# megvii-research/basedet

Hardware: AMD Instinct MI355X
Metric: images/sec training RetinaNet-R50-FPN 1333x800 (higher is better)
Workload: dtype bf16; 1 GPU; retinanet_r50_800x1344 train step (fwd+bwd+allreduce+SGD), DummyLoader boxes, random-init weights, inputs resident in HBM; per_gpu_batch=16, global_batch=16, parallelism=dp1

## Files before the change

### basedet_amd/_lib.py

```python
import ctypes as C
import os

import torch

_HERE = os.path.dirname(os.path.abspath(__file__))
LIB_PATH = os.environ.get("BASEDET_HIP_LIB") or os.path.join(_HERE, "lib", "libbasedet_hip.so")

BD_MAX_SEGS = 8
ABI_VERSION = 118
EPI_RELU, EPI_ADD_BEFORE, EPI_ADD_AFTER, EPI_MASK, EPI_SPARSE = 1, 2, 4, 8, 16


class BasedetHipError(RuntimeError):
    pass


class ConvDesc(C.Structure):
    _fields_ = [
        ("N", C.c_int32), ("Cin", C.c_int32), ("Cout", C.c_int32), ("R", C.c_int32), ("S", C.c_int32),
        ("stride", C.c_int32), ("pad", C.c_int32), ("nseg", C.c_int32),
        ("Hi", C.c_int32 * BD_MAX_SEGS), ("Wi", C.c_int32 * BD_MAX_SEGS),
        ("Ho", C.c_int32 * BD_MAX_SEGS), ("Wo", C.c_int32 * BD_MAX_SEGS),
        ("in_off", C.c_int32 * BD_MAX_SEGS), ("out_off", C.c_int32 * BD_MAX_SEGS),
        ("in_pix_per_img", C.c_int32), ("out_pix_per_img", C.c_int32),
# ... 98 lines not shown
    "bd_box_encode": (_I, [_P, _P, _L, _P, _P, _P, _P]),
    "bd_box_decode": (_I, [_P, _P, _L, _P, _P, _P, _P]),
    "bd_retina_assign_encode": (_I, [_P, _I, _P, _P, _I, _I, _F, _F, _I, _P, _P, _P, _P, _P, _P, _P, _Z, _P]),
    "bd_fcos_assign": (_I, [_P, _I, _P, _P, _P, _I, _F, _P, _P, _I, _I, _P, _P, _P, _P, _P]),
    "bd_ota_assign_workspace_bytes": (_Z, [_I, _I]),
    "bd_ota_assign": (_I, [_P, _I, _P, _P, _I, _P, _I, _I, _P, _P, _P, _I, _I, _F, _F, _F, _F, _I, _P, _P, _P, _P, _P, _Z, _P]),
    "bd_ota_sinkhorn_workspace_bytes": (_Z, [_I, _I, _I]),
    "bd_ota_assign_sinkhorn": (_I, [_P, _I, _P, _P, _I, _P, _I, _I, _P, _P, _P, _I, _I, _F, _F, _F, _F, _I, _F, _I, _P, _P, _P, _P, _P, _Z, _P]),
    "bd_freeanchor_workspace_bytes": (_Z, [_I, _I, _I, _I]),
    "bd_freeanchor_loss_fwd_bwd": (_I, [_P, _I, _P, _I, _I, _P, _I, _I, _P, _P, _I, _I, _P, _P, _F, _I, _F, _F, _F, _F, _P, _P, _P, _P, _Z, _P]),
    "bd_atss_assign_workspace_bytes": (_Z, [_I, _I]),
    "bd_atss_assign": (_I, [_P, _I, _P, _P, _I, _I, _F, _P, _P, _I, _I, _P, _P, _P, _P, _P, _Z, _P]),
    "bd_nms_workspace_bytes": (_Z, [_I]),
    "bd_batched_nms": (_I, [_P, _P, _P, _I, _F, _I, _P, _P, _P, _Z, _P]),
    "bd_focal_loss_fwd_bwd": (_I, [_P, _P, _L, _I, _I, _F, _F, _P, _I, _F, _P, _P, _I, _P]),
    "bd_smooth_l1_fwd_bwd": (_I, [_P, _P, _P, _L, _I, _I, _F, _P, _I, _F, _P, _P, _P]),
    "bd_loss_grid_cap": (_I, []),
    "bd_iou_ltrb_fwd_bwd": (_I, [_P, _P, _P, _P, _L, _I, _P, _F, _P, _P, _P]),
    "bd_bce_logits_fwd_bwd": (_I, [_P, _I, _I, _P, _P, _L, _P, _P, _P, _P]),
    "bd_groupnorm_workspace_bytes": (_Z, [_I, _I, _I, _L]),
    "bd_groupnorm_fwd": (_I, [_P, _P, _P, _I, _I, _P, _P, _L, _I, _F, _I, _P, _P, _P, _Z, _P]),
    "bd_conv2d_fwd_gnstats_bytes": (_Z, [_D]),
    "bd_conv2d_fwd_gnstats": (_I, [_D, _P, _P, _P, _P, _P, _Z, _P]),
    "bd_groupnorm_fwd_parts": (_I, [_D, _P, _P, _P, _P, _F, _I, _P, _P, _P]),
    "bd_groupnorm_bwd": (_I, [_P, _P, _P, _P, _P, _I, _I, _P, _P, _L, _I, _I, _P, _P, _P, _I, _P, _Z, _P]),
    "bd_bn_workspace_bytes": (_Z, [_L, _I]),
    "bd_bn_stats_fwd": (_I, [_P, _I, _L, _L, _L, _I, _F, _F, _P, _P, _P, _P, _P, _P, _Z, _P]),
    "bd_bn_apply_act_fwd": (_I, [_P, _L, _L, _P, _P, _P, _P, _P, _L, _L, _P, _L, _L, _I, _L, _I, _I, _P]),
    "bd_bn_bwd_reduce": (_I, [_P, _L, _L, _P, _L, _L, _P, _P, _I, _L, _I, _P, _P, _P, _Z, _P]),
    "bd_bn_bwd_apply": (_I, [_P, _L, _L, _P, _L, _L, _P, _P, _P, _P, _P, _P, _P, _L, _L, _I, _L, _I, _P]),
    "bd_bn_silu_fwd": (_I, [_P, _L, _L, _P, _P, _P, _P, _P, _L, _L, _I, _L, _I, _P]),
# ... 151 lines not shown
```

### basedet_amd/csrc/conv3x3_pp.hip

```cpp
#include "conv3x3_pp128_body.h"

namespace {

constexpr int PH = 4, PW = 16, IH = PH + 2, IW = PW + 2;
constexpr int NPATCH = 4;
constexpr int XROWS = NPATCH * IH * IW;
constexpr int X_PITCH = 144;
constexpr int X_BYTES = XROWS * X_PITCH;
constexpr int XPASSES = 7;
constexpr int TILE_CO = 256;
constexpr int W_SLOT = TILE_CO * 128;
constexpr int NSLOT = 3;
constexpr int W_BYTES = NSLOT * W_SLOT;
constexpr int GTAB_TILES = 16;
constexpr int GTAB_BYTES = GTAB_TILES * NPATCH * 32;
constexpr int LDS_BYTES = W_BYTES + X_BYTES + TILE_CO * 4 + GTAB_BYTES;
constexpr int MAX_SEG = BD_MAX_SEGS;
constexpr int TAIL_CO = 64;

struct PSeg { int patch_start, H, W, pw, src_off, dst_off; float inv_pw; };

struct PParams {
    const bf16_raw* src;
    const bf16_raw* w;
// ... 607 lines not shown
    }
    if (!SPARSE && blockIdx.x == 0 && threadIdx.x == 0) bd_clk_mark(g_pp_clk, true);
#ifdef BD_PP_STAMP
    if (st_on) { g_pp_stamp[63] = __builtin_amdgcn_s_memrealtime(); g_pp_stamp[61] = __builtin_amdgcn_s_memtime(); }
    if (threadIdx.x == 0 && blockIdx.x < 1024) { asm volatile("s_waitcnt vmcnt(0)" ::: "memory"); g_pp_span[2 * blockIdx.x + 1] = __builtin_amdgcn_s_memrealtime(); }
#endif
}

}

BD_KNOB int g_pp_tail_split = 1;
BD_KNOB int g_pp_persistent = 1;
extern BD_KNOB int g_patch_pp;
int bd_gskip_patches(const bd_conv_desc* d, int ph, int pw);
void bd_gskip_fill(const bd_conv_desc* d, int side, const void* t, const int* live_in, int* map, hipStream_t stream);
void bd_gskip_scan(const bd_conv_desc* d, const void* g, int ph, int pw, int* mask, hipStream_t stream);
void bd_gskip_compact(const bd_conv_desc* d, int ph, int pw, const int* mask, int* live, int* list, int* count, hipStream_t stream);

extern "C" size_t bd_conv2d_dgrad_gskip_bytes(const bd_conv_desc* d) {
    if (!d || d->nseg < 1 || d->nseg > BD_MAX_SEGS || !(d->R == 3 && d->S == 3 && d->stride == 1 && d->pad == 1)) return 0;
    return ((size_t)3 * bd_gskip_patches(d, PH, PW) + 4) * sizeof(int);
}

static bool pp_sparse_epilogue(int flags, const void* add, const void* dst) {
    const bool in_place = (flags & BD_EPI_ADD_BEFORE) && add && add == dst;
    return !(flags & BD_EPI_ADD_AFTER) && (!((flags & BD_EPI_ADD_BEFORE) && add) || (in_place && !(flags & BD_EPI_MASK)));
}

bool bd_conv3x3_pp_maps_ok(const bd_conv_desc* d, int flags, const void* add, const void* dst) {
    if (g_patch_pp < 2 || !(d->R == 3 && d->S == 3 && d->stride == 1 && d->pad == 1)) return false;
    if (d->Cout % 8 != 0 || d->Cin <= 128 || d->Cin % 8 != 0) return false;
    if ((long long)d->N * d->out_pix_per_img * d->Cout * 2 >= 0x7fffffffll || (long long)d->N * d->in_pix_per_img >= 0x7fffffffll ||
// ... 80 lines not shown
        (void)hipFuncSetAttribute(reinterpret_cast<const void*>(&conv3x3_pp_kernel<0, false, true>), hipFuncAttributeMaxDynamicSharedMemorySize,
                                  LDS_BYTES));
    bd_note_kernel("conv3x3_pp_kernel");
    if (sparse) {
        const int tot = p.total_patches;
        p.sp_keep_dead = in_place ? 1 : 0;
        p.sp_stride = tot;
        if (d->gskip_gmap) {
            BdGskipMap gm;
            bd_gskip_map_layout(d, 0, &gm);
            const int* m = (const int*)d->gskip_gmap;
            p.sp_hdr = m; p.sp_live = m + gm.live; p.sp_list = m + gm.list;
        } else {
            int* mk = (int*)d->gskip_ws;
            p.sp_live = mk + tot; p.sp_list = mk + 2 * tot; p.sp_count = mk + 3 * tot;
            bd_gskip_scan(d, src, PH, PW, mk, stream);
            bd_gskip_compact(d, PH, PW, mk, mk + tot, mk + 2 * tot, mk + 3 * tot, stream);
        }
        if (d->gskip_dxmap) {
            BdGskipMap xm;
            bd_gskip_map_layout(d, 1, &xm);
            p.sp_ohdr = (int*)d->gskip_dxmap; p.sp_olist = p.sp_ohdr + xm.list;
            p.sp_clean = d->gskip_dx_clean ? 1 : 0;
        }
        hipLaunchKernelGGL((conv3x3_pp_kernel<1, false, true>), dim3(p.main_grid), dim3(512), LDS_BYTES, stream, p);
        if (d->gskip_dxmap) bd_gskip_fill(d, 1, dst, p.sp_live, (int*)d->gskip_dxmap, stream);
    } else if (fsparse) {
        const int tot = p.total_patches;
        BdFwdMap fm;
        bd_fwd_map_layout(d, &fm);
        int* m = (int*)d->fwd_map;
        p.sp_hdr = m; p.sp_live = m + fm.live; p.sp_list = m + fm.list; p.sp_stride = tot;
// ... 63 lines not shown
```

### basedet_amd/csrc/gskip.hip

```cpp
#include "common.h"

namespace {

enum { GS_ANY = 1, GS_TOP = 2, GS_BOT = 4, GS_LEFT = 8, GS_RIGHT = 16, GS_TL = 32, GS_TR = 64, GS_BL = 128, GS_BR = 256 };

struct GsSeg { int patch_start, H, W, pw, off; };

struct GsParams {
    const bf16_raw* g;
    int* mask;
    int C, ppi, ph, pw_px, nseg, patches_per_img, total;
    GsSeg seg[BD_MAX_SEGS];
};

__device__ __forceinline__ int gs_level(const GsParams& p, int rem) {
    int s = 0;
#pragma unroll
    for (int k = 1; k < BD_MAX_SEGS; ++k)
        if (k < p.nseg && rem >= p.seg[k].patch_start) s = k;
    return s;
}

__global__ __launch_bounds__(256) void gskip_scan_kernel(const GsParams p) {
    __shared__ int sbits;
    const int tid = threadIdx.x;
    const int pid = blockIdx.x;
    const int n = pid / p.patches_per_img, rem = pid - n * p.patches_per_img;
    const int s = gs_level(p, rem);
    const int H = p.seg[s].H, W = p.seg[s].W, pwn = p.seg[s].pw;
    const int local = rem - p.seg[s].patch_start, by = local / pwn, bx = local - by * pwn;
    const int y0 = by * p.ph, x0 = bx * p.pw_px;
    const int cpp = p.C >> 3;
    const int items = p.ph * p.pw_px * cpp;
    const long long img = (long long)n * p.ppi + p.seg[s].off;
    if (tid == 0) sbits = 0;
    __syncthreads();
    int bits = 0;
    constexpr int U = 8;
    for (int b = 0; b < items; b += 256 * U) {
// ... 16 lines not shown
        }
#pragma unroll
        for (int k = 0; k < U; ++k) {
            if (pix[k] >= 0 && (v[k][0] | v[k][1] | v[k][2] | v[k][3])) {
                const int py = pix[k] / p.pw_px, pxx = pix[k] - py * p.pw_px;
                const bool t = py == 0, bo = py == p.ph - 1, l = pxx == 0, r = pxx == p.pw_px - 1;
                bits |= GS_ANY | (t ? GS_TOP : 0) | (bo ? GS_BOT : 0) | (l ? GS_LEFT : 0) | (r ? GS_RIGHT : 0) | (t && l ? GS_TL : 0) |
                        (t && r ? GS_TR : 0) | (bo && l ? GS_BL : 0) | (bo && r ? GS_BR : 0);
            }
        }
    }
#pragma unroll
    for (int m = 32; m >= 1; m >>= 1) bits |= __shfl_xor(bits, m, 64);
    if ((tid & 63) == 0 && bits) atomicOr(&sbits, bits);
    __syncthreads();
    if (tid == 0) p.mask[pid] = sbits;
}

template <bool FRESH>
__device__ __forceinline__ int gs_mask(const int* m, int i) {
    if (FRESH) return __hip_atomic_load(m + i, __ATOMIC_RELAXED, __HIP_MEMORY_SCOPE_AGENT);
    return m[i];
}

template <bool FRESH>
__device__ __forceinline__ void gs_compact_body(const GsParams& p, int* live, int* list, int* count, int* wsum) {
    constexpr int KP = 8;
    const int tid = threadIdx.x, wv = tid >> 6, ln = tid & 63;
    int base = 0;
    for (int c0 = 0; c0 < p.total; c0 += 1024 * KP) {
        int lv[KP];
#pragma unroll
        for (int j = 0; j < KP; ++j) {
            const int q = c0 + tid * KP + j;
            lv[j] = 0;
            if (q < p.total) {
                const int n = q / p.patches_per_img, rem = q - n * p.patches_per_img;
                const int s = gs_level(p, rem);
                const int pwn = p.seg[s].pw, rows = (p.seg[s].H + p.ph - 1) / p.ph;
                const int local = rem - p.seg[s].patch_start, by = local / pwn, bx = local - by * pwn;
                const int* m = p.mask + (long long)n * p.patches_per_img + p.seg[s].patch_start;
                const bool up = by > 0, dn = by + 1 < rows, lf = bx > 0, rt = bx + 1 < pwn;
                int v = gs_mask<FRESH>(m, by * pwn + bx) & GS_ANY;
                if (up) v |= gs_mask<FRESH>(m, (by - 1) * pwn + bx) & GS_BOT;
                if (dn) v |= gs_mask<FRESH>(m, (by + 1) * pwn + bx) & GS_TOP;
// ... 7 lines not shown
            }
        }
        int cnt = 0;
#pragma unroll
        for (int j = 0; j < KP; ++j) cnt += lv[j];
        int inc = cnt;
#pragma unroll
        for (int o = 1; o < 64; o <<= 1) {
            const int y = __shfl_up(inc, o, 64);
            if (ln >= o) inc += y;
        }
        if (ln == 63) wsum[wv] = inc;
        __syncthreads();
        int off = base + inc - cnt, tot = 0;
#pragma unroll
        for (int w = 0; w < 16; ++w) {
            off += w < wv ? wsum[w] : 0;
            tot += wsum[w];
        }
#pragma unroll
        for (int j = 0; j < KP; ++j) {
            const int q = c0 + tid * KP + j;
            if (q < p.total) live[q] = lv[j];
            if (lv[j]) list[off++] = q;
        }
        base += tot;
        __syncthreads();
    }
    if (tid == 0) *count = base;
}

__global__ __launch_bounds__(1024) void gskip_compact_kernel(const GsParams p, int* live, int* list, int* count) {
    __shared__ int wsum[16];
    gs_compact_body<false>(p, live, list, count, wsum);
}

enum { GM_HDR = 8 };

struct GmSeg { int H, W, off, s4, s8, ss; };

struct GmParams {
    const bf16_raw* t;
    const int* live_in;
    int* map;
    int C, ppi, nseg, pi4, pi8, pis, tot4, tot8;
    GmSeg seg[BD_MAX_SEGS];
};

__global__ __launch_bounds__(1024) void gskip_fill_kernel(const GmParams p, const GsParams cp, int total) {
// ... 190 lines not shown

int bd_gskip_patches(const bd_conv_desc* d, int ph, int pw) {
    return gs_params(d, ph, pw).total;
}

void bd_gskip_scan(const bd_conv_desc* d, const void* g, int ph, int pw, int* mask, hipStream_t stream) {
    GsParams p = gs_params(d, ph, pw);
    p.g = (const bf16_raw*)g; p.mask = mask;
    if (p.total > 0) hipLaunchKernelGGL(gskip_scan_kernel, dim3(p.total), dim3(256), 0, stream, p);
}

void bd_gskip_compact(const bd_conv_desc* d, int ph, int pw, const int* mask, int* live, int* list, int* count, hipStream_t stream) {
    GsParams p = gs_params(d, ph, pw);
    p.mask = const_cast<int*>(mask);
    hipLaunchKernelGGL(gskip_compact_kernel, dim3(1), dim3(1024), 0, stream, p, live, list, count);
}

void bd_gskip_map_layout(const bd_conv_desc* d, int side, BdGskipMap* out) {
    const int p4 = gs_params(d, 4, 16, side).total, p8 = gs_params(d, 8, 8, side).total;
    out->p4 = p4; out->p8 = p8;
    out->m4 = GM_HDR; out->m8 = GM_HDR + p4; out->live = out->m8 + p8; out->list = out->live + p4;
    out->ints = (size_t)GM_HDR + (size_t)4 * p4 + p8;
}

extern "C" size_t bd_conv2d_gskip_map_bytes(const bd_conv_desc* d, int of_dx) {
    if (!d || d->nseg < 1 || d->nseg > BD_MAX_SEGS || !(d->R == 3 && d->S == 3 && d->stride == 1 && d->pad == 1)) return 0;
    BdGskipMap m;
    bd_gskip_map_layout(d, of_dx ? 1 : 0, &m);
    return m.ints * sizeof(int);
}
// ... 85 lines not shown
```

### basedet_amd/csrc/losses.hip

```cpp
#include <utility>
#include <vector>

#include "common.h"

namespace {

__device__ __forceinline__ float load_norm(const void* norm, int is_float) {
    float v = is_float ? *reinterpret_cast<const float*>(norm) : (float)*reinterpret_cast<const int*>(norm);
    return fmaxf(v, 1.f);
}

__device__ __forceinline__ float block_sum_256(float v, float* red) {
    v = wave_sum(v);
    if ((threadIdx.x & 63) == 0) red[threadIdx.x >> 6] = v;
    __syncthreads();
    return red[0] + red[1] + red[2] + red[3];
}

__device__ __forceinline__ float log1p_small(float e, float log_rounded) {
    return e < 0x1p-10f ? e * (1.f - e * (0.5f - e * 0.33333334f)) : log_rounded;
}

__device__ __forceinline__ void focal_elem(float x, bool t, float alpha, float gamma, float& loss, float& grad) {
    const float e = __expf(-fabsf(x));
// ... 424 lines not shown
        partial[2 * r] = (lse - bf2f(rp[l])) * gs;
        float sb = 0.f;
        if (l > 0) {
            for (int k = 0; k < 4; ++k) {
                const float x = bf2f(rp[box_off + (l - 1) * 4 + k]) - targets[(long long)r * 4 + k];
                const float ax = fabsf(x);
                if (beta < 1e-5f) sb += ax;
                else if (ax < beta) sb += 0.5f * x * x / beta;
                else sb += ax - 0.5f * beta;
            }
        }
        partial[2 * r + 1] = sb * gs;
    }
}

__global__ __launch_bounds__(256) void loss_finalize_kernel(const float* __restrict__ partial, int n, int slots, float* __restrict__ loss) {
    __shared__ float red[4];
    for (int k = 0; k < slots; ++k) {
        float a = 0.f;
        for (int b = threadIdx.x; b < n; b += 256) a += partial[(long long)b * slots + k];
        const float s = block_sum_256(a, red);
        if (threadIdx.x == 0) loss[k] += s;
        __syncthreads();
    }
}

constexpr int LOSS_GRID_CAP = 4096;

inline int loss_grid(long long n) {
    long long g = (n + 255) / 256;
    if (g < 1) g = 1;
    return (int)(g < LOSS_GRID_CAP ? g : LOSS_GRID_CAP);
}

}

static float* loss_partials(hipStream_t stream, size_t floats) {
// ... 12 lines not shown
    }
    if (b->n < floats) {
        if (b->p) (void)hipFree(b->p);
        b->p = nullptr; b->n = 0;
        const size_t n = floats < 8192 ? 8192 : floats;
        if (hipMalloc((void**)&b->p, n * sizeof(float)) != hipSuccess) return nullptr;
        b->n = n;
    }
    return b->p;
}

#define BD_LOSS_PARTIALS(var, stream, floats, name)                                                                          \
    float* var = loss_partials((hipStream_t)(stream), (size_t)(floats));                                                     \
    BD_REQUIRE(var != nullptr, name ": cannot allocate %zu bytes of partial-sum scratch", (size_t)(floats) * sizeof(float))

static void loss_finalize(const float* partial, int n, int slots, float* loss, bd_stream_t stream) {
    hipLaunchKernelGGL(loss_finalize_kernel, dim3(1), dim3(256), 0, (hipStream_t)stream, partial, n, slots, loss);
}

extern "C" int bd_focal_loss_fwd_bwd(const void* logits, const int32_t* labels, int64_t rows, int K, int ld, float alpha, float gamma,
                                     const void* norm, int norm_is_float, float grad_scale, float* loss_sum, void* dlogits, int general,
                                     bd_stream_t stream) {
    BD_REQUIRE(logits && labels && norm && loss_sum && dlogits, "focal_loss: null pointer");
    BD_REQUIRE(K > 0 && ld % 8 == 0 && ld >= K && ld - K < 8, "focal_loss: the row stride ld=%d must be K=%d rounded up to a multiple of 8", ld, K);
    if (rows == 0) return BD_OK;
    const int grid = loss_grid(rows * (ld / 8));
    BD_LOSS_PARTIALS(part, stream, grid, "focal_loss");
    if (gamma == 2.f && !general)
        hipLaunchKernelGGL(focal_g2_kernel, dim3(grid), dim3(256), 0, (hipStream_t)stream,
                           (const bf16_raw*)logits, labels, (long long)rows, K, ld, alpha, norm, norm_is_float, grad_scale, part,
                           (bf16_raw*)dlogits);
    else
        hipLaunchKernelGGL(focal_kernel, dim3(grid), dim3(256), 0, (hipStream_t)stream,
                           (const bf16_raw*)logits, labels, (long long)rows, K, ld, alpha, gamma, norm, norm_is_float, grad_scale,
                           part, (bf16_raw*)dlogits);
    loss_finalize(part, grid, 1, loss_sum, stream);
    BD_CHECK_LAUNCH("bd_focal_loss_fwd_bwd");
    return BD_OK;
}

extern "C" int bd_smooth_l1_fwd_bwd(const void* pred, const float* target, const int32_t* labels, int64_t pixels, int A,
                                    int ld, float beta, const void* norm, int norm_is_float, float weight, float* loss_sum,
                                    void* dpred, bd_stream_t stream) {
    BD_REQUIRE(pred && target && labels && norm && loss_sum && dpred, "smooth_l1: null pointer");
    BD_REQUIRE(A > 0 && ld >= 4 * A && ld % 4 == 0, "smooth_l1: ld=%d must be a multiple of 4 and >= 4*A", ld);
    if (pixels == 0) return BD_OK;
    const int grid = loss_grid(pixels * (ld / 4));
    BD_LOSS_PARTIALS(part, stream, grid, "smooth_l1");
    hipLaunchKernelGGL(smooth_l1_kernel, dim3(grid), dim3(256), 0, (hipStream_t)stream,
                       (const bf16_raw*)pred, target, labels, (long long)pixels, A, ld, beta, norm, norm_is_float, weight,
                       part, (bf16_raw*)dpred);
    loss_finalize(part, grid, 1, loss_sum, stream);
    BD_CHECK_LAUNCH("bd_smooth_l1_fwd_bwd");
    return BD_OK;
}

extern "C" int bd_loss_grid_cap(void) { return LOSS_GRID_CAP; }

extern "C" int bd_iou_ltrb_fwd_bwd(const void* pred, const float* target, const float* weight, const int32_t* labels,
                                   int64_t rows, int loss_type, const float* norm, float loss_weight, float* loss_sum, void* dpred,
                                   bd_stream_t stream) {
    BD_REQUIRE(pred && target && labels && norm && loss_sum && dpred, "iou_ltrb: null pointer");
    BD_REQUIRE(loss_type >= 0 && loss_type <= 3, "iou_ltrb: loss_type %d (0 iou, 1 linear_iou, 2 giou, 3 square_iou)", loss_type);
    if (rows == 0) return BD_OK;
    const int grid = loss_grid(rows);
    BD_LOSS_PARTIALS(part, stream, grid, "iou_ltrb");
    auto kernel = loss_type == IOU_LT_GIOU ? iou_ltrb_kernel<IOU_LT_GIOU> : loss_type == IOU_LT_LINEAR ? iou_ltrb_kernel<IOU_LT_LINEAR>
// ... 50 lines not shown
```

### basedet_amd/models/fpn_base.py

```python
import math

import numpy as np
import torch

from .. import ops
from ..data.raw import AffineImageBatch, RawImageBatch
from ..ops import Geom
from ..streams import SideStreams, fork, join
from . import params as P
from .. import comm as _comm
from .engine import ConvLayer, DeconvLayer, FCLayer, ParamArena, TrainableStem
from .fp8_scaling import Fp8GradScaler, initial_grad_scale
from .live_norm import BatchNormState, LiveNorms
from .plan_arena import PlanArena, _Carver, _Plan, _round_up
from .wgrad_sched import WgradScheduler


class VecParam:

    def __init__(self, name, numel):
        self.name, self.numel = name, numel
        self.w = self.g = None

    def reserve(self, arena):
# ... 801 lines not shown
        s["num"].zero_()
        ops.nms_batched(s["boxes"], s["sc"], s["labels"], t.IOU_THRESHOLD, max_out, s["keep"], s["num"], s["nms_ws"])
        ob = torch.empty((N, max_out, 4), dtype=torch.float32, device=dev)
        osc = torch.empty((N, max_out), dtype=torch.float32, device=dev)
        ol = torch.empty((N, max_out), dtype=torch.int32, device=dev)
        ops.det_finalize(s["boxes"], s["sc"], s["labels"], s["keep"], s["num"], max_out, info, ob, osc, ol)
        outs = []
        for i, n in enumerate(s["num"].tolist()):
            if n == 0:
                e = torch.zeros((0,))
                outs.append(Container(boxes=e, box_scores=e, box_labels=e))
            else:
                outs.append(Container(boxes=Boxes(ob[i, :n]), box_scores=osc[i, :n], box_labels=ol[i, :n]))
        return outs

    def _wgrad(self, conv, x, g, gin, gout, ws, cws=None, x8=None, g8=None):
        self.wgrads.run(conv, x, g, gin, gout, ws, cws, x8, g8)

    def _begin_wgrads(self):
        self.wgrads.begin()

    def _flush_wgrads(self):
        self.wgrads.flush()

    def _join_wgrads(self):
        self.wgrads.join()

    def _norm_backward(self, n, g, gg, pl):
        y, gy, geo = pl.norm_y[n.name], pl.norm_gy[n.name], pl.norm_geo[n.name]
        ops.bn_bwd_reduce(g, gg, y, geo, n.mean, n.inv_std, n.C, n.g_gamma, n.g_beta, pl.bn_ws)
        return ops.bn_bwd_apply(g, gg, y, geo, n.mean, n.inv_std, n.gamma, n.g_gamma, n.g_beta, n.sums[0], gy, geo, n.C)

# ... 186 lines not shown
```

### basedet_amd/models/retinanet.py

```python
import torch

from .. import ops
from ..streams import fork, join
from ..utils.registry import registers
from . import params as P
from .engine import PaddedClsConv
from .fpn_base import FPNDetector, _round_up


@registers.models.register()
class RetinaNet(FPNDetector):
    READS_MATCHER = True

    @staticmethod
    def init_params(cfg, seed=0):
        return P.init_retinanet_params(cfg, seed)

    @classmethod
    def check_config(cls, cfg):
        super().check_config(cfg)
        cls.check_anchor_config(cfg, matcher=cls.READS_MATCHER)
        if not cfg.MODEL.HEAD.get("WITH_NORM", True):
            raise ValueError("MODEL.HEAD.WITH_NORM = False is not supported for the RetinaNet family: only True (the default) is implemented")

# ... 3 lines not shown
        self.num_anchors = len(m.ANCHOR.SCALES[0]) * len(m.ANCHOR.RATIOS[0])
        nc = m.HEAD.NUM_CONVS
        self.cls_tower = [add(f"head.cls_subnet.{2 * i}", ch, ch, 3, 1, 1, bias=True) for i in range(nc)]
        self.box_tower = [add(f"head.bbox_subnet.{2 * i}", ch, ch, 3, 1, 1, bias=True) for i in range(nc)]
        A, K = self.num_anchors, self.num_classes
        self.cls_score = self.convs["head.cls_score"] = PaddedClsConv("head.cls_score", ch, A, K, 3, 1, 1, self.device)
        self.cls_ld = self.cls_score.cls_ld
        self.box_ld = _round_up(A * 4, 8)
        self.bbox_pred = add("head.bbox_pred", ch, A * 4, 3, 1, 1, bias=True, cout_pad=self.box_ld)
        if bool(m.get("SPARSE_BOX_BWD", True)) and m.get("WEIGHT_DTYPE", "bf16") == "bf16":
            for c in self.box_tower + [self.bbox_pred]:
                c.gskip = True
        self.sparse_chain = bool(m.get("SPARSE_BOX_CHAIN", True))
        self.sparse_box_fwd = (bool(m.get("SPARSE_BOX_FWD", True)) and type(self) is RetinaNet and nc >= 1 and nc <= 8
                               and all(c.gskip for c in self.box_tower + [self.bbox_pred]))
        self._build_base_anchors()

    def _head_convs(self):
        return self.cls_tower + self.box_tower + [self.cls_score, self.bbox_pred]

    def _plan_head(self, pl):
        ch = self.fpn_ch
        N = pl.N
        C = pl._carve
        bf = torch.bfloat16

        def act(g, c):
            return C.empty((g.pixels, c), bf)

        nc = len(self.cls_tower)
# ... 7 lines not shown
        pl.g_tower = [[act(pl.pyr, ch) for _ in range(nc)] for _ in range(2)]
        pl.g_map = None
        if self.sparse_chain and all(c.gskip for c in self.box_tower + [self.bbox_pred]):
            nb = ops.conv2d_gskip_map_bytes(self.box_tower[0].desc(pl.pyr, pl.pyr))
            if nb:
                pl.g_map = [C.empty(((nb + 3) // 4,), torch.int32) for _ in range(nc)]
        pl.chain_epoch = None
        pl.f_map = None
        if self.sparse_box_fwd:
            nb = ops.fwd_live_map_bytes(self.box_tower[0].desc(pl.pyr, pl.pyr))
            if nb:
                pl.f_map = [C.empty(((nb + 3) // 4,), torch.int32) for _ in range(nc)]
        pl.fwd_epoch = None
        pl.fwd_skip = None
        pl.fwd_skipped = False
        tw = lambda: C.empty((pl.pyr.pixels, ch), torch.uint8)
        pl.cls_act8 = [tw() if c.fp8 else None for c in self.cls_tower]
        pl.box_act8 = [tw() if c.fp8 else None for c in self.box_tower]
        tg = self.fp8_grad_twins
        pl.g_tower8 = [[tw() if (c.fp8_dgrad and tg) else None for c in tower] for tower in (self.cls_tower, self.box_tower)]
        pl.g_P8 = tw() if (tg and all(t[0].fp8_dgrad for t in (self.cls_tower, self.box_tower))) else None
        self._plan_anchors(pl)
        tot = pl.A_total
        pl.labels = C.empty((N, tot), torch.int32)
        pl.match_idx = C.empty((N, tot), torch.int32)
        pl.gt_offsets = C.empty((N, tot, 4), torch.float32)
        pl.num_fg = C.zeros((1,), torch.int32)
        pl.loss_buf = C.zeros((2,), torch.float32)

    def head_forward(self, pl):
        concurrent = bool(self.cfg.MODEL.get("HEAD_TOWERS_CONCURRENT", True)) and self.weight_dtype != "fp8_e4m3"
        side = self.streams.aux() if concurrent else None
        skip, pl.fwd_skip = pl.fwd_skip, None
        if skip is not None and side is None:
            join(self.streams.aux_stream)
        if skip is None:
            pl.fwd_epoch = None
        pl.fwd_skipped = skip is not None
        with fork(side):
            t, t8 = pl.P, getattr(pl, "P8", None)
            for i, (c, a, a8) in enumerate(zip(self.box_tower, pl.box_act, pl.box_act8)):
                if skip is not None:
                    c.forward(t, pl.pyr, pl.pyr, a, relu=True, fwd_map=pl.f_map[i], fwd_clean=skip[0])
                else:
                    c.forward(t, pl.pyr, pl.pyr, a, relu=True, x8=t8, y8=a8)
                t, t8 = a, a8
            self.bbox_pred.forward(t, pl.pyr, pl.pyr, pl.offsets, x8=t8)
        t, t8 = pl.P, getattr(pl, "P8", None)
        for c, a, a8 in zip(self.cls_tower, pl.cls_act, pl.cls_act8):
            c.forward(t, pl.pyr, pl.pyr, a, relu=True, x8=t8, y8=a8); t, t8 = a, a8
        self.cls_score.forward(t, pl.pyr, pl.pyr, pl.logits, x8=t8)
        join(side)

    def get_losses(self, inputs):
        assert self.training
        pre = self.pre_process(inputs)
        pl = pre["plan"]
        self._cur = pl
        m = self.cfg.MODEL
        gt = pre["gt_boxes"]
        num_gt = pre["img_info"][:, 4].to(torch.int32).contiguous()
        N, Gmax = gt.shape[0], gt.shape[1]
        ws = self._scratch("assign", N * Gmax * 4).view(torch.float32)
        thr = m.MATCHER.THRESHOLDS
        side = self.streams.aux() if m.get("ASSIGN_ON_SIDE_STREAM", True) else None
        with fork(side):
            ops.retina_assign_encode(pl.anchors, gt, num_gt, thr[0], thr[1], m.MATCHER.ALLOW_LOW_QUALITY, m.BOX_REG.MEAN,
                                     m.BOX_REG.STD, pl.labels, pl.match_idx, pl.gt_offsets, pl.num_fg, ws)
            if pl.f_map is not None and self.streams.aux() is not None:
                clean = pl.fwd_epoch == self.plan_arena.epoch
                pl.fwd_epoch = self.plan_arena.epoch
                ops.fwd_live_maps(self.box_tower[0].desc(pl.pyr, pl.pyr), pl.labels, self.num_anchors, pl.f_map[::-1], reset=not clean)
                pl.fwd_skip = (clean,)
        self.network_forward(pl)
        join(side)
        pl.loss_buf.zero_()
        rows = N * pl.A_total
        ops.focal_loss_fwd_bwd(pl.logits, pl.labels, rows, self.num_classes, m.LOSSES.FOCAL_LOSS_ALPHA,
                               m.LOSSES.FOCAL_LOSS_GAMMA, pl.num_fg, 1.0, pl.loss_buf[0:1], pl.d_logits, ld=self.cls_ld)
        ops.smooth_l1_fwd_bwd(pl.offsets, pl.gt_offsets, pl.labels, pl.pyr.pixels, self.num_anchors, self.box_ld,
                              m.LOSSES.SMOOTH_L1_BETA, pl.num_fg, m.LOSSES.REG_LOSS_WEIGHT, pl.loss_buf[1:2], pl.d_offsets)
        cls_loss, reg_loss = pl.loss_buf[0], pl.loss_buf[1]
        return {"total_loss": cls_loss + reg_loss, "cls_loss": cls_loss, "reg_loss": reg_loss}

    def head_backward(self, pl, ws, cws):
        pyr = pl.pyr
        for ti, (tower, acts, pred, dpred) in enumerate(((self.cls_tower, pl.cls_act, self.cls_score, pl.d_logits),
                                                         (self.box_tower, pl.box_act, self.bbox_pred, pl.d_offsets))):
            gbuf, g8 = pl.g_tower[ti], pl.g_tower8[ti]
            n = len(tower)
            maps = pl.g_map if (ti == 1 and self.sparse_chain and all(c.gskip for c in tower + [pred])) else None
            if ti == 1:
                clean = maps is not None and pl.chain_epoch == self.plan_arena.epoch
                pl.chain_epoch = self.plan_arena.epoch if maps is not None else None
                if maps is not None:
                    pred.set_chain(None, maps[n - 1], clean)
                    for i in range(n):
                        tower[i].set_chain(maps[i], maps[i - 1] if i > 0 else None, clean)
            gs = tower[n - 1].grad_scale
            self._wgrad(pred, acts[-1], dpred, pyr, pyr, ws, cws)
            tw = g8[n - 1] if pred.dgrad_writes_twin(pyr, pyr) else None
            if not pred.dgrad(dpred, pyr, pyr, gbuf[n - 1], mask=acts[-1], dx8=tw, q_scale=gs):
                tw = None
# ... 3 lines not shown
                x8 = (act8[i - 1] if i > 0 else pl.P8) if tw is not None else None
                self._wgrad(tower[i], x, gbuf[i], pyr, pyr, ws, cws, x8=x8, g8=tw)
                if i > 0:
                    nxt = g8[i - 1] if tower[i].dgrad_writes_twin(pyr, pyr) else None
                    wrote = tower[i].dgrad(gbuf[i], pyr, pyr, gbuf[i - 1], mask=acts[i - 1], g8=tw, dx8=nxt, q_scale=tower[i - 1].grad_scale)
                    tw = nxt if wrote else None
                else:
                    wrote_p = tower[i].dgrad(gbuf[i], pyr, pyr, pl.g_P, first=(ti == 0), g8=tw,
                                             dx8=pl.g_P8 if tower[i].dgrad_writes_twin(pyr, pyr) else None,
                                             q_scale=self.output[self.fpn_stages[0]].grad_scale)
        for c in self.box_tower + [self.bbox_pred]:
            c.set_chain()
        pl.g_P8_ready = pl.g_P8 is not None and bool(wrote_p)

    def _debug_head(self, pl, out, lvl):
        if getattr(pl, "fwd_skipped", False):
            t = pl.P
            for c, a in zip(self.box_tower, pl.box_act):
                c.forward(t, pl.pyr, pl.pyr, a, relu=True); t = a
            self.bbox_pred.forward(t, pl.pyr, pl.pyr, pl.offsets)
            pl.fwd_skipped = False
            pl.fwd_epoch = None
        for i in range(pl.pyr.nlev):
            for k in range(len(self.cls_tower)):
                out[f"cls{k}_{i}"] = lvl(pl.cls_act[k], i)
                out[f"box{k}_{i}"] = lvl(pl.box_act[k], i)
            lg = lvl(pl.logits, i)
            out[f"logits_{i}"] = self.cls_score.real_logits(lg.permute(0, 2, 3, 1)).permute(0, 3, 1, 2).contiguous()
            out[f"offs_{i}"] = lvl(pl.offsets, i, self.num_anchors * 4)

    def inference_batch(self, inputs):
        assert not self.training
        pre = self.pre_process(inputs)
        pl = pre["plan"]
        self.network_forward(pl)
        K, A = self.num_classes, self.num_anchors
        m = self.cfg.MODEL
        return self._detect(pl.N, [h * w * A for h, w in pl.sizes], K, 0, pre["img_info"], logits=pl.logits, anchors=pl.anchors,
                            offsets=pl.offsets, off_ld=self.box_ld, A=A, mean=m.BOX_REG.MEAN, std=m.BOX_REG.STD, cls_ld=self.cls_ld)
```

### basedet_amd/models/wgrad_sched.py

```python
import torch

from .. import ops
from ..streams import fork, join


class WgradScheduler:
    def __init__(self, device, queue_mode, streams):
        self.device = torch.device(device)
        self.streams = streams
        self.queue_mode = queue_mode
        self.queue = None
        self.need = {}
        self.arena = None
        self.off = self.pending = self.peak = 0

    def run(self, conv, x, g, gin, gout, ws, cws=None, x8=None, g8=None):
        q = None
        if self.queue_mode != "layer" and self.device.type == "cuda" and not (conv.fp8_wgrad and x8 is not None and g8 is not None):
            key = (conv.name, gin.N, tuple(gin.H), tuple(gin.W), tuple(gout.H), tuple(gout.W))
            need = self.need.get(key)
            if need is None:
                need = self.need[key] = (conv.wgrad_ws_bytes(gin, gout) + 255) // 256 * 256
            off = self.off
            self.off = off + need
            arena = self.arena
            if arena is not None and off + need <= arena.numel() * 4:
                ws = arena[off // 4: (off + need) // 4]
                self.pending += need
                if self.queue is None:
                    self.queue = ops.WgradQueue()
                q = self.queue
        with fork(self.streams.wgrad()):
            conv.wgrad(x, g, gin, gout, ws, cws, x8=x8, g8=g8, queue=q)
        if q is not None and isinstance(self.queue_mode, int) and self.pending >= self.queue_mode:
            self.flush()

    def begin(self):
        if self.queue is None or not self.queue.pending():
            self.off = self.pending = 0

    def flush(self):
        self.peak = max(self.peak, self.off)
        self.off = self.pending = 0
        q = self.queue
        if q is None or not q.pending():
            return
        with fork(self.streams.wgrad(), wait=False):
# ... 10 lines not shown
```

### basedet_amd/ops.py

```python
import ctypes as C
from dataclasses import dataclass, field
from typing import List, Optional

import torch

from . import _lib
from ._lib import ConvDesc, EPI_ADD_AFTER, EPI_ADD_BEFORE, EPI_MASK, EPI_RELU, EPI_SPARSE, check, f32arr, i32arr, ptr, stream_ptr


@dataclass
class Geom:
    N: int
    H: List[int]
    W: List[int]
    off: List[int] = field(default_factory=list)
    pix_per_img: int = 0

    def __post_init__(self):
        if not self.off:
            o = 0
            self.off = []
            for h, w in zip(self.H, self.W):
                self.off.append(o)
                o += h * w
# ... 705 lines not shown


def det_select(logits, B, rows, K, seg_start, seg_rows, k, min_score, out_idx, out_score, out_cnt, ws, ctr=None, ctr_ld=1, ctr_off=0,
               ld=None):
    check(L().bd_det_select(ptr(logits), int(K if ld is None else ld), ptr(ctr), ctr_ld, ctr_off, B, rows, K, len(seg_start),
                            i32arr(seg_start), i32arr(seg_rows), k, float(min_score), ptr(out_idx), ptr(out_score), ptr(out_cnt), ptr(ws),
                            ws.numel() * ws.element_size(), stream_ptr()), "bd_det_select")


def focal_loss_fwd_bwd(logits, labels, rows, K, alpha, gamma, norm, grad_scale, loss_sum, dlogits, general=False, ld=None):
    check(L().bd_focal_loss_fwd_bwd(ptr(logits), ptr(labels), rows, K, int(K if ld is None else ld), float(alpha), float(gamma), ptr(norm),
                                    int(norm.dtype == torch.float32), float(grad_scale), ptr(loss_sum), ptr(dlogits), int(bool(general)),
                                    stream_ptr()), "bd_focal_loss_fwd_bwd")


def smooth_l1_fwd_bwd(pred, target, labels, pixels, A, ld, beta, norm, weight, loss_sum, dpred):
    check(L().bd_smooth_l1_fwd_bwd(ptr(pred), ptr(target), ptr(labels), pixels, A, ld, float(beta), ptr(norm),
                                   int(norm.dtype == torch.float32), float(weight), ptr(loss_sum), ptr(dpred), stream_ptr()),
          "bd_smooth_l1_fwd_bwd")


def loss_grid_cap():
    return int(L().bd_loss_grid_cap())


IOU_LOSS_TYPES = {"iou": 0, "linear_iou": 1, "giou": 2, "square_iou": 3}


def iou_ltrb_fwd_bwd(pred, target, weight, labels, rows, loss_type, norm, loss_weight, loss_sum, dpred):
    check(L().bd_iou_ltrb_fwd_bwd(ptr(pred), ptr(target), ptr(weight), ptr(labels), rows, int(loss_type), ptr(norm), float(loss_weight),
                                  ptr(loss_sum), ptr(dpred), stream_ptr()), "bd_iou_ltrb_fwd_bwd")


# ... 398 lines not shown
```

### basedet_amd/streams.py

```python
from contextlib import contextmanager

import torch


@contextmanager
def fork(stream, wait=True):
    if stream is None:
        yield
        return
    if wait:
        stream.wait_stream(torch.cuda.current_stream())
    with torch.cuda.stream(stream):
        yield


def join(stream):
    if stream is not None:
        torch.cuda.current_stream().wait_stream(stream)


class SideStreams:

    def __init__(self, device):
        self.enabled = True
        on_gpu = torch.cuda.is_available() and torch.device(device).type == "cuda"
        self.wgrad_stream = torch.cuda.Stream() if on_gpu else None
        self.aux_stream = torch.cuda.Stream() if on_gpu else None

    def wgrad(self):
        return self.wgrad_stream if self.enabled else None

    def aux(self):
# ... 6 lines not shown
```

### include/basedet_hip.h

```cpp
#ifndef BASEDET_HIP_H
#define BASEDET_HIP_H

#include <stddef.h>
#include <stdint.h>

#ifdef __cplusplus
extern "C" {
#endif

#define BD_OK 0
#define BD_EINVAL (-1)
#define BD_ELAUNCH (-2)
#define BD_EWORKSPACE (-3)

#define BD_MAX_SEGS 8

#define BD_EPI_RELU 1
#define BD_EPI_ADD_BEFORE 2
#define BD_EPI_ADD_AFTER 4
#define BD_EPI_MASK 8
#define BD_EPI_SPARSE 16

typedef void* bd_stream_t;

// ... 230 lines not shown

size_t bd_nms_workspace_bytes(int n);
int bd_batched_nms(const float* boxes, const float* scores, const int32_t* idxs, int n, float iou_thresh,
                   int max_output, int32_t* keep, int32_t* num_keep, void* ws, size_t ws_bytes,
                   bd_stream_t stream);


int bd_focal_loss_fwd_bwd(const void* logits, const int32_t* labels, int64_t rows, int K, int ld, float alpha, float gamma,
                          const void* norm, int norm_is_float, float grad_scale, float* loss_sum, void* dlogits, int general,
                          bd_stream_t stream);

int bd_loss_grid_cap(void);

int bd_smooth_l1_fwd_bwd(const void* pred, const float* target, const int32_t* labels, int64_t pixels, int A,
                         int ld, float beta, const void* norm, int norm_is_float, float weight, float* loss_sum,
                         void* dpred, bd_stream_t stream);

int bd_iou_ltrb_fwd_bwd(const void* pred, const float* target, const float* weight, const int32_t* labels, int64_t rows, int loss_type,
                        const float* norm, float loss_weight, float* loss_sum, void* dpred, bd_stream_t stream);

int bd_bce_logits_fwd_bwd(const void* pred, int ld, int off, const float* target, const int32_t* labels, int64_t rows,
                          const float* norm, float* loss_sum, void* dpred, bd_stream_t stream);


size_t bd_groupnorm_workspace_bytes(int N, int L, int C, int64_t pix_per_img);
int bd_groupnorm_fwd(const void* y, const float* gamma, const float* beta, int N, int L, const int32_t* lvl_off_host,
                     const int32_t* lvl_cnt_host, int64_t pix_per_img, int C, float eps, int relu, float* stats,
                     void* z, void* ws, size_t ws_bytes, bd_stream_t stream);
size_t bd_conv2d_fwd_gnstats_bytes(const bd_conv_desc* d);
int bd_conv2d_fwd_gnstats(const bd_conv_desc* d, const void* x, const void* w_packed, const float* bias, void* y, float* part,
                          size_t part_bytes, bd_stream_t stream);
// ... 264 lines not shown
```

Baseline: 720.6 images/sec.

## Run box-branch loss and dgrad chain concurrently on side stream during forward

When the sparse box forward path is active, the box head's smooth-L1 loss and its dgrad chain are launched on the side stream right after the box forward, overlapping with the cls tower forward and focal loss. Events mark each dgrad stage so the wgrads can wait on them instead of the whole stream. The gskip scan and compact kernels are also fused into one launch using a last-block ticket counter. The cost is more cross-stream event logic, an overwrite mode for the loss finalize, and a per-stream ticket buffer that adds ordering risk.

```diff
diff --git a/basedet_amd/_lib.py b/basedet_amd/_lib.py
--- a/basedet_amd/_lib.py
+++ b/basedet_amd/_lib.py
@@ -136,7 +136,7 @@
     "bd_nms_workspace_bytes": (_Z, [_I]),
     "bd_batched_nms": (_I, [_P, _P, _P, _I, _F, _I, _P, _P, _P, _Z, _P]),
     "bd_focal_loss_fwd_bwd": (_I, [_P, _P, _L, _I, _I, _F, _F, _P, _I, _F, _P, _P, _I, _P]),
-    "bd_smooth_l1_fwd_bwd": (_I, [_P, _P, _P, _L, _I, _I, _F, _P, _I, _F, _P, _P, _P]),
+    "bd_smooth_l1_fwd_bwd": (_I, [_P, _P, _P, _L, _I, _I, _F, _P, _I, _F, _P, _P, _I, _P]),
     "bd_loss_grid_cap": (_I, []),
     "bd_iou_ltrb_fwd_bwd": (_I, [_P, _P, _P, _P, _L, _I, _P, _F, _P, _P, _P]),
     "bd_bce_logits_fwd_bwd": (_I, [_P, _I, _I, _P, _P, _L, _P, _P, _P, _P]),
diff --git a/basedet_amd/csrc/conv3x3_pp.hip b/basedet_amd/csrc/conv3x3_pp.hip
--- a/basedet_amd/csrc/conv3x3_pp.hip
+++ b/basedet_amd/csrc/conv3x3_pp.hip
@@ -645,8 +645,8 @@
 extern BD_KNOB int g_patch_pp;
 int bd_gskip_patches(const bd_conv_desc* d, int ph, int pw);
 void bd_gskip_fill(const bd_conv_desc* d, int side, const void* t, const int* live_in, int* map, hipStream_t stream);
-void bd_gskip_scan(const bd_conv_desc* d, const void* g, int ph, int pw, int* mask, hipStream_t stream);
-void bd_gskip_compact(const bd_conv_desc* d, int ph, int pw, const int* mask, int* live, int* list, int* count, hipStream_t stream);
+void bd_gskip_scan_compact(const bd_conv_desc* d, const void* g, int ph, int pw, int* mask, int* live, int* list, int* count,
+                           hipStream_t stream);
 
 extern "C" size_t bd_conv2d_dgrad_gskip_bytes(const bd_conv_desc* d) {
     if (!d || d->nseg < 1 || d->nseg > BD_MAX_SEGS || !(d->R == 3 && d->S == 3 && d->stride == 1 && d->pad == 1)) return 0;
@@ -757,8 +757,7 @@
         } else {
             int* mk = (int*)d->gskip_ws;
             p.sp_live = mk + tot; p.sp_list = mk + 2 * tot; p.sp_count = mk + 3 * tot;
-            bd_gskip_scan(d, src, PH, PW, mk, stream);
-            bd_gskip_compact(d, PH, PW, mk, mk + tot, mk + 2 * tot, mk + 3 * tot, stream);
+            bd_gskip_scan_compact(d, src, PH, PW, mk, mk + tot, mk + 2 * tot, mk + 3 * tot, stream);
         }
         if (d->gskip_dxmap) {
             BdGskipMap xm;
diff --git a/basedet_amd/csrc/gskip.hip b/basedet_amd/csrc/gskip.hip
--- a/basedet_amd/csrc/gskip.hip
+++ b/basedet_amd/csrc/gskip.hip
@@ -1,3 +1,7 @@
+#include <mutex>
+#include <utility>
+#include <vector>
+
 #include "common.h"
 
 namespace {
@@ -21,8 +25,8 @@
     return s;
 }
 
-__global__ __launch_bounds__(256) void gskip_scan_kernel(const GsParams p) {
-    __shared__ int sbits;
+__device__ __forceinline__ int gs_scan_patch(const GsParams& p, int* sbits_p) {
+    int& sbits = *sbits_p;
     const int tid = threadIdx.x;
     const int pid = blockIdx.x;
     const int n = pid / p.patches_per_img, rem = pid - n * p.patches_per_img;
@@ -69,7 +73,13 @@
     for (int m = 32; m >= 1; m >>= 1) bits |= __shfl_xor(bits, m, 64);
     if ((tid & 63) == 0 && bits) atomicOr(&sbits, bits);
     __syncthreads();
-    if (tid == 0) p.mask[pid] = sbits;
+    return sbits;
+}
+
+__global__ __launch_bounds__(256) void gskip_scan_kernel(const GsParams p) {
+    __shared__ int sbits;
+    const int w = gs_scan_patch(p, &sbits);
+    if (threadIdx.x == 0) p.mask[blockIdx.x] = w;
 }
 
 template <bool FRESH>
@@ -78,12 +88,12 @@
     return m[i];
 }
 
-template <bool FRESH>
+template <bool FRESH, int NT = 1024>
 __device__ __forceinline__ void gs_compact_body(const GsParams& p, int* live, int* list, int* count, int* wsum) {
     constexpr int KP = 8;
     const int tid = threadIdx.x, wv = tid >> 6, ln = tid & 63;
     int base = 0;
-    for (int c0 = 0; c0 < p.total; c0 += 1024 * KP) {
+    for (int c0 = 0; c0 < p.total; c0 += NT * KP) {
         int lv[KP];
 #pragma unroll
         for (int j = 0; j < KP; ++j) {
@@ -121,7 +131,7 @@
         __syncthreads();
         int off = base + inc - cnt, tot = 0;
 #pragma unroll
-        for (int w = 0; w < 16; ++w) {
+        for (int w = 0; w < NT / 64; ++w) {
             off += w < wv ? wsum[w] : 0;
             tot += wsum[w];
         }
@@ -140,6 +150,22 @@
 __global__ __launch_bounds__(1024) void gskip_compact_kernel(const GsParams p, int* live, int* list, int* count) {
     __shared__ int wsum[16];
     gs_compact_body<false>(p, live, list, count, wsum);
+}
+
+__global__ __launch_bounds__(256) void gskip_scan_compact_kernel(const GsParams p, int* live, int* list, int* count, int* ticket) {
+    __shared__ int sbits, slast;
+    __shared__ int wsum[16];
+    const int w = gs_scan_patch(p, &sbits);
+    if (threadIdx.x == 0) {
+        __hip_atomic_store(p.mask + blockIdx.x, w, __ATOMIC_RELAXED, __HIP_MEMORY_SCOPE_AGENT);
+        asm volatile("s_waitcnt vmcnt(0)" ::: "memory");
+        slast = __hip_atomic_fetch_add(ticket, 1, __ATOMIC_RELAXED, __HIP_MEMORY_SCOPE_AGENT) == (int)gridDim.x - 1;
+    }
+    __syncthreads();
+    if (!slast) return;
+    __builtin_amdgcn_fence(__ATOMIC_ACQUIRE, "agent");
+    gs_compact_body<true, 256>(p, live, list, count, wsum);
+    if (threadIdx.x == 0) __hip_atomic_store(ticket, 0, __ATOMIC_RELAXED, __HIP_MEMORY_SCOPE_AGENT);
 }
 
 enum { GM_HDR = 8 };
@@ -360,6 +386,34 @@
     GsParams p = gs_params(d, ph, pw);
     p.mask = const_cast<int*>(mask);
     hipLaunchKernelGGL(gskip_compact_kernel, dim3(1), dim3(1024), 0, stream, p, live, list, count);
+}
+
+static int* gs_ticket(hipStream_t stream) {
+    static std::mutex mu;
+    static std::vector<std::pair<std::pair<int, hipStream_t>, int*>> words;
+    int dev = 0;
+    if (hipGetDevice(&dev) != hipSuccess) return nullptr;
+    std::lock_guard<std::mutex> g(mu);
+    for (auto& e : words)
+        if (e.first.first == dev && e.first.second == stream) return e.second;
+    int* w = nullptr;
+    if (hipMalloc((void**)&w, 64) != hipSuccess) return nullptr;
+    if (hipMemset(w, 0, 64) != hipSuccess) { (void)hipFree(w); return nullptr; }
+    words.push_back({{dev, stream}, w});
+    return w;
+}
+
+void bd_gskip_scan_compact(const bd_conv_desc* d, const void* g, int ph, int pw, int* mask, int* live, int* list, int* count,
+                           hipStream_t stream) {
+    GsParams p = gs_params(d, ph, pw);
+    p.g = (const bf16_raw*)g; p.mask = mask;
+    int* ticket = p.total > 0 ? gs_ticket(stream) : nullptr;
+    if (!ticket) {
+        bd_gskip_scan(d, g, ph, pw, mask, stream);
+        bd_gskip_compact(d, ph, pw, mask, live, list, count, stream);
+        return;
+    }
+    hipLaunchKernelGGL(gskip_scan_compact_kernel, dim3(p.total), dim3(256), 0, stream, p, live, list, count, ticket);
 }
 
 void bd_gskip_map_layout(const bd_conv_desc* d, int side, BdGskipMap* out) {
diff --git a/basedet_amd/csrc/losses.hip b/basedet_amd/csrc/losses.hip
--- a/basedet_amd/csrc/losses.hip
+++ b/basedet_amd/csrc/losses.hip
@@ -462,13 +462,14 @@
     }
 }
 
-__global__ __launch_bounds__(256) void loss_finalize_kernel(const float* __restrict__ partial, int n, int slots, float* __restrict__ loss) {
+__global__ __launch_bounds__(256) void loss_finalize_kernel(const float* __restrict__ partial, int n, int slots, float* __restrict__ loss,
+                                                            int overwrite) {
     __shared__ float red[4];
     for (int k = 0; k < slots; ++k) {
         float a = 0.f;
         for (int b = threadIdx.x; b < n; b += 256) a += partial[(long long)b * slots + k];
         const float s = block_sum_256(a, red);
-        if (threadIdx.x == 0) loss[k] += s;
+        if (threadIdx.x == 0) loss[k] = (overwrite ? 0.f : loss[k]) + s;
         __syncthreads();
     }
 }
@@ -511,8 +512,8 @@
     float* var = loss_partials((hipStream_t)(stream), (size_t)(floats));                                                     \
     BD_REQUIRE(var != nullptr, name ": cannot allocate %zu bytes of partial-sum scratch", (size_t)(floats) * sizeof(float))
 
-static void loss_finalize(const float* partial, int n, int slots, float* loss, bd_stream_t stream) {
-    hipLaunchKernelGGL(loss_finalize_kernel, dim3(1), dim3(256), 0, (hipStream_t)stream, partial, n, slots, loss);
+static void loss_finalize(const float* partial, int n, int slots, float* loss, bd_stream_t stream, int overwrite = 0) {
+    hipLaunchKernelGGL(loss_finalize_kernel, dim3(1), dim3(256), 0, (hipStream_t)stream, partial, n, slots, loss, overwrite);
 }
 
 extern "C" int bd_focal_loss_fwd_bwd(const void* logits, const int32_t* labels, int64_t rows, int K, int ld, float alpha, float gamma,
@@ -538,16 +539,21 @@
 
 extern "C" int bd_smooth_l1_fwd_bwd(const void* pred, const float* target, const int32_t* labels, int64_t pixels, int A,
                                     int ld, float beta, const void* norm, int norm_is_float, float weight, float* loss_sum,
-                                    void* dpred, bd_stream_t stream) {
+                                    void* dpred, int overwrite, bd_stream_t stream) {
     BD_REQUIRE(pred && target && labels && norm && loss_sum && dpred, "smooth_l1: null pointer");
     BD_REQUIRE(A > 0 && ld >= 4 * A && ld % 4 == 0, "smooth_l1: ld=%d must be a multiple of 4 and >= 4*A", ld);
-    if (pixels == 0) return BD_OK;
+    if (pixels == 0 && !overwrite) return BD_OK;
     const int grid = loss_grid(pixels * (ld / 4));
     BD_LOSS_PARTIALS(part, stream, grid, "smooth_l1");
+    if (pixels == 0) {
+        loss_finalize(part, 0, 1, loss_sum, stream, 1);
+        BD_CHECK_LAUNCH("bd_smooth_l1_fwd_bwd");
+        return BD_OK;
+    }
     hipLaunchKernelGGL(smooth_l1_kernel, dim3(grid), dim3(256), 0, (hipStream_t)stream,
                        (const bf16_raw*)pred, target, labels, (long long)pixels, A, ld, beta, norm, norm_is_float, weight,
                        part, (bf16_raw*)dpred);
-    loss_finalize(part, grid, 1, loss_sum, stream);
+    loss_finalize(part, grid, 1, loss_sum, stream, overwrite ? 1 : 0);
     BD_CHECK_LAUNCH("bd_smooth_l1_fwd_bwd");
     return BD_OK;
 }
diff --git a/basedet_amd/models/fpn_base.py b/basedet_amd/models/fpn_base.py
--- a/basedet_amd/models/fpn_base.py
+++ b/basedet_amd/models/fpn_base.py
@@ -839,8 +839,8 @@
                 outs.append(Container(boxes=Boxes(ob[i, :n]), box_scores=osc[i, :n], box_labels=ol[i, :n]))
         return outs
 
-    def _wgrad(self, conv, x, g, gin, gout, ws, cws=None, x8=None, g8=None):
-        self.wgrads.run(conv, x, g, gin, gout, ws, cws, x8, g8)
+    def _wgrad(self, conv, x, g, gin, gout, ws, cws=None, x8=None, g8=None, after=None):
+        self.wgrads.run(conv, x, g, gin, gout, ws, cws, x8, g8, after=after)
 
     def _begin_wgrads(self):
         self.wgrads.begin()
diff --git a/basedet_amd/models/retinanet.py b/basedet_amd/models/retinanet.py
--- a/basedet_amd/models/retinanet.py
+++ b/basedet_amd/models/retinanet.py
@@ -1,7 +1,7 @@
 import torch
 
 from .. import ops
-from ..streams import fork, join
+from ..streams import fork, join, mark
 from ..utils.registry import registers
 from . import params as P
 from .engine import PaddedClsConv
@@ -41,6 +41,9 @@
         self.sparse_chain = bool(m.get("SPARSE_BOX_CHAIN", True))
         self.sparse_box_fwd = (bool(m.get("SPARSE_BOX_FWD", True)) and type(self) is RetinaNet and nc >= 1 and nc <= 8
                                and all(c.gskip for c in self.box_tower + [self.bbox_pred]))
+        self.box_bwd_concurrent = bool(m.get("BOX_BWD_CONCURRENT", True)) and self.sparse_box_fwd and self.sparse_chain
+        self._box_marks = {}
+        self._box_bwd_open = None
         self._build_base_anchors()
 
     def _head_convs(self):
@@ -78,6 +81,8 @@
         pl.fwd_epoch = None
         pl.fwd_skip = None
         pl.fwd_skipped = False
+        pl.box_bwd_go = False
+        pl.box_bwd = None
         tw = lambda: C.empty((pl.pyr.pixels, ch), torch.uint8)
         pl.cls_act8 = [tw() if c.fp8 else None for c in self.cls_tower]
         pl.box_act8 = [tw() if c.fp8 else None for c in self.box_tower]
@@ -101,6 +106,8 @@
         if skip is None:
             pl.fwd_epoch = None
         pl.fwd_skipped = skip is not None
+        go, pl.box_bwd_go = pl.box_bwd_go, False
+        go = go and skip is not None and side is not None and pl.g_map is not None and self.streams.wgrad() is not None
         with fork(side):
             t, t8 = pl.P, getattr(pl, "P8", None)
             for i, (c, a, a8) in enumerate(zip(self.box_tower, pl.box_act, pl.box_act8)):
@@ -110,14 +117,45 @@
                     c.forward(t, pl.pyr, pl.pyr, a, relu=True, x8=t8, y8=a8)
                 t, t8 = a, a8
             self.bbox_pred.forward(t, pl.pyr, pl.pyr, pl.offsets, x8=t8)
+            if go:
+                self._box_bwd_launch(pl)
         t, t8 = pl.P, getattr(pl, "P8", None)
         for c, a, a8 in zip(self.cls_tower, pl.cls_act, pl.cls_act8):
             c.forward(t, pl.pyr, pl.pyr, a, relu=True, x8=t8, y8=a8); t, t8 = a, a8
         self.cls_score.forward(t, pl.pyr, pl.pyr, pl.logits, x8=t8)
-        join(side)
+        if pl.box_bwd is None:
+            join(side)
+
+    def _box_bwd_launch(self, pl):
+        m = self.cfg.MODEL
+        pyr, n = pl.pyr, len(self.box_tower)
+        tower, pred, acts, gbuf, maps = self.box_tower, self.bbox_pred, pl.box_act, pl.g_tower[1], pl.g_map
+        mk = self._box_marks
+        ops.smooth_l1_fwd_bwd(pl.offsets, pl.gt_offsets, pl.labels, pyr.pixels, self.num_anchors, self.box_ld, m.LOSSES.SMOOTH_L1_BETA,
+                              pl.num_fg, m.LOSSES.REG_LOSS_WEIGHT, pl.loss_buf[1:2], pl.d_offsets, overwrite=True)
+        mk["loss"] = mark(mk.get("loss"))
+        clean = pl.chain_epoch == self.plan_arena.epoch
+        pl.chain_epoch = self.plan_arena.epoch
+        pred.set_chain(None, maps[n - 1], clean)
+        for i in range(n):
+            tower[i].set_chain(maps[i], maps[i - 1] if i > 0 else None, clean)
+        pred.dgrad(pl.d_offsets, pyr, pyr, gbuf[n - 1], mask=acts[-1])
+        mk[n - 1] = mark(mk.get(n - 1))
+        for i in range(n - 1, 0, -1):
+            tower[i].dgrad(gbuf[i], pyr, pyr, gbuf[i - 1], mask=acts[i - 1])
+            mk[i - 1] = mark(mk.get(i - 1))
+        pl.box_bwd = mk
+        self._box_bwd_open = pl
+
+    def _box_bwd_close(self):
+        pl, self._box_bwd_open = self._box_bwd_open, None
+        if pl is not None:
+            pl.box_bwd = None
+            join(self.streams.aux_stream)
 
     def get_losses(self, inputs):
         assert self.training
+        self._box_bwd_close()
         pre = self.pre_process(inputs)
         pl = pre["plan"]
         self._cur = pl
@@ -136,10 +174,18 @@
                 pl.fwd_epoch = self.plan_arena.epoch
                 ops.fwd_live_maps(self.box_tower[0].desc(pl.pyr, pl.pyr), pl.labels, self.num_anchors, pl.f_map[::-1], reset=not clean)
                 pl.fwd_skip = (clean,)
+                pl.box_bwd_go = self.box_bwd_concurrent
         self.network_forward(pl)
+        rows = N * pl.A_total
+        if pl.box_bwd is not None:
+            join(pl.box_bwd["loss"])
+            pl.loss_buf[0:1].zero_()
+            ops.focal_loss_fwd_bwd(pl.logits, pl.labels, rows, self.num_classes, m.LOSSES.FOCAL_LOSS_ALPHA,
+                                   m.LOSSES.FOCAL_LOSS_GAMMA, pl.num_fg, 1.0, pl.loss_buf[0:1], pl.d_logits, ld=self.cls_ld)
+            cls_loss, reg_loss = pl.loss_buf[0], pl.loss_buf[1]
+            return {"total_loss": cls_loss + reg_loss, "cls_loss": cls_loss, "reg_loss": reg_loss}
         join(side)
         pl.loss_buf.zero_()
-        rows = N * pl.A_total
         ops.focal_loss_fwd_bwd(pl.logits, pl.labels, rows, self.num_classes, m.LOSSES.FOCAL_LOSS_ALPHA,
                                m.LOSSES.FOCAL_LOSS_GAMMA, pl.num_fg, 1.0, pl.loss_buf[0:1], pl.d_logits, ld=self.cls_ld)
         ops.smooth_l1_fwd_bwd(pl.offsets, pl.gt_offsets, pl.labels, pl.pyr.pixels, self.num_anchors, self.box_ld,
@@ -147,10 +193,26 @@
         cls_loss, reg_loss = pl.loss_buf[0], pl.loss_buf[1]
         return {"total_loss": cls_loss + reg_loss, "cls_loss": cls_loss, "reg_loss": reg_loss}
 
+    def _box_bwd_join(self, pl, chain, ws, cws):
+        pyr, n = pl.pyr, len(self.box_tower)
+        tower, acts, gbuf = self.box_tower, pl.box_act, pl.g_tower[1]
+        self._wgrad(self.bbox_pred, acts[-1], pl.d_offsets, pyr, pyr, ws, cws, after=chain["loss"])
+        for i in range(n - 1, -1, -1):
+            self._wgrad(tower[i], acts[i - 1] if i > 0 else pl.P, gbuf[i], pyr, pyr, ws, cws, after=chain[i])
+        self._box_bwd_open = None
+        join(self.streams.aux_stream)
+        return tower[0].dgrad(gbuf[0], pyr, pyr, pl.g_P, first=False,
+                              dx8=pl.g_P8 if tower[0].dgrad_writes_twin(pyr, pyr) else None,
+                              q_scale=self.output[self.fpn_stages[0]].grad_scale)
+
     def head_backward(self, pl, ws, cws):
         pyr = pl.pyr
+        chain, pl.box_bwd = pl.box_bwd, None
         for ti, (tower, acts, pred, dpred) in enumerate(((self.cls_tower, pl.cls_act, self.cls_score, pl.d_logits),
                                                          (self.box_tower, pl.box_act, self.bbox_pred, pl.d_offsets))):
+            if ti == 1 and chain is not None:
+                wrote_p = self._box_bwd_join(pl, chain, ws, cws)
+                break
             gbuf, g8 = pl.g_tower[ti], pl.g_tower8[ti]
             n = len(tower)
             maps = pl.g_map if (ti == 1 and self.sparse_chain and all(c.gskip for c in tower + [pred])) else None
@@ -184,6 +246,8 @@
         pl.g_P8_ready = pl.g_P8 is not None and bool(wrote_p)
 
     def _debug_head(self, pl, out, lvl):
+        if self._box_bwd_open is not None:
+            join(self.streams.aux_stream)
         if getattr(pl, "fwd_skipped", False):
             t = pl.P
             for c, a in zip(self.box_tower, pl.box_act):
@@ -201,6 +265,7 @@
 
     def inference_batch(self, inputs):
         assert not self.training
+        self._box_bwd_close()
         pre = self.pre_process(inputs)
         pl = pre["plan"]
         self.network_forward(pl)
diff --git a/basedet_amd/models/wgrad_sched.py b/basedet_amd/models/wgrad_sched.py
--- a/basedet_amd/models/wgrad_sched.py
+++ b/basedet_amd/models/wgrad_sched.py
@@ -14,7 +14,7 @@
         self.arena = None
         self.off = self.pending = self.peak = 0
 
-    def run(self, conv, x, g, gin, gout, ws, cws=None, x8=None, g8=None):
+    def run(self, conv, x, g, gin, gout, ws, cws=None, x8=None, g8=None, after=None):
         q = None
         if self.queue_mode != "layer" and self.device.type == "cuda" and not (conv.fp8_wgrad and x8 is not None and g8 is not None):
             key = (conv.name, gin.N, tuple(gin.H), tuple(gin.W), tuple(gout.H), tuple(gout.W))
@@ -30,7 +30,7 @@
                 if self.queue is None:
                     self.queue = ops.WgradQueue()
                 q = self.queue
-        with fork(self.streams.wgrad()):
+        with fork(self.streams.wgrad(), wait=after is None, after=after):
             conv.wgrad(x, g, gin, gout, ws, cws, x8=x8, g8=g8, queue=q)
         if q is not None and isinstance(self.queue_mode, int) and self.pending >= self.queue_mode:
             self.flush()
diff --git a/basedet_amd/ops.py b/basedet_amd/ops.py
--- a/basedet_amd/ops.py
+++ b/basedet_amd/ops.py
@@ -743,9 +743,10 @@
                                     stream_ptr()), "bd_focal_loss_fwd_bwd")
 
 
-def smooth_l1_fwd_bwd(pred, target, labels, pixels, A, ld, beta, norm, weight, loss_sum, dpred):
+def smooth_l1_fwd_bwd(pred, target, labels, pixels, A, ld, beta, norm, weight, loss_sum, dpred, overwrite=False):
     check(L().bd_smooth_l1_fwd_bwd(ptr(pred), ptr(target), ptr(labels), pixels, A, ld, float(beta), ptr(norm),
-                                   int(norm.dtype == torch.float32), float(weight), ptr(loss_sum), ptr(dpred), stream_ptr()),
+                                   int(norm.dtype == torch.float32), float(weight), ptr(loss_sum), ptr(dpred), int(bool(overwrite)),
+                                   stream_ptr()),
           "bd_smooth_l1_fwd_bwd")
 
 
diff --git a/basedet_amd/streams.py b/basedet_amd/streams.py
--- a/basedet_amd/streams.py
+++ b/basedet_amd/streams.py
@@ -4,18 +4,31 @@
 
 
 @contextmanager
-def fork(stream, wait=True):
+def fork(stream, wait=True, after=None):
     if stream is None:
+        join(after)
         yield
         return
     if wait:
         stream.wait_stream(torch.cuda.current_stream())
+    if after is not None:
+        stream.wait_event(after)
     with torch.cuda.stream(stream):
         yield
 
 
+def mark(event=None):
+    event = torch.cuda.Event() if event is None else event
+    event.record(torch.cuda.current_stream())
+    return event
+
+
 def join(stream):
-    if stream is not None:
+    if stream is None:
+        return
+    if isinstance(stream, torch.cuda.Event):
+        torch.cuda.current_stream().wait_event(stream)
+    else:
         torch.cuda.current_stream().wait_stream(stream)
 
 
diff --git a/include/basedet_hip.h b/include/basedet_hip.h
--- a/include/basedet_hip.h
+++ b/include/basedet_hip.h
@@ -268,7 +268,7 @@
 
 int bd_smooth_l1_fwd_bwd(const void* pred, const float* target, const int32_t* labels, int64_t pixels, int A,
                          int ld, float beta, const void* norm, int norm_is_float, float weight, float* loss_sum,
-                         void* dpred, bd_stream_t stream);
+                         void* dpred, int overwrite, bd_stream_t stream);
 
 int bd_iou_ltrb_fwd_bwd(const void* pred, const float* target, const float* weight, const int32_t* labels, int64_t rows, int loss_type,
                         const float* norm, float loss_weight, float* loss_sum, void* dpred, bd_stream_t stream);
```

After: 726.4 images/sec (median of 6 runs). Within noise of the previous version (+0.8%).
